# StefanHeng/Symbolic-Music-Generation

Measured on AMD Instinct MI355X. Metric: train tokens/sec (TransfoXL seq2048 bf16), whole job, higher is better.
Workload: dtype bf16; 1 GPU; TransfoXL 12L/768d H12 dh64 F3072 T=2048 M=2048 V=1190 cutoffs=[] (SURVEY C3, mode R: fresh zero mems); per_gpu_batch=64, global_batch=64, seq_len=2048, mem_len=2048, parallelism=dp1

## Files before the change

symbolic_music_generation_amd/csrc/relattn_fwd.hip:

```cpp
#include <type_traits>
#include "common.h"
#include "musicxl_internal.h"

namespace {

typedef __attribute__((ext_vector_type(8))) __bf16 mfma_bf16x8;
typedef __attribute__((address_space(3))) bf16x4 lds_bf16x4;

struct RelAttnP {
    const bf16_t *q, *k, *v, *rd;
    const float *rwb, *rrb;
    bf16_t* out;
    float* lse;
    int B, T, H, M, Kc;
    long long q_bs, kv_bs, o_bs;
    int q_rs, kv_rs, rd_rs, o_rs;
    float scale_log2e;
    bf16_t* oph;
    float* mph;
    int oph_all;
    char* ph_rec;
};

constexpr int QB = 128;
constexpr int KT = 64;
constexpr int GS = 100;
constexpr float NEG_BIG = -1.0e30f;

__device__ __forceinline__ int floordiv(int a, int b) { return (a >= 0) ? a / b : -((-a + b - 1) / b); }

template <int DH> struct Geo {
    static constexpr int KS = DH / 16;
    static constexpr int EB = (DH + 31) / 32;
    static constexpr int VW = EB * 32;
    static constexpr int ROWB = DH * 2;
    static constexpr int VROWB = VW * 2;
    static constexpr int CH = DH / 8;
    static constexpr int VCH = VW / 8;
    static constexpr int K_BYTES = KT * ROWB;
    static constexpr int V_BYTES = KT * VROWB;
    static constexpr int R_BYTES = 256 * ROWB;
    static constexpr int G_BYTES = 4 * 32 * GS * 2;
    static constexpr int SMEM = K_BYTES + V_BYTES + R_BYTES + G_BYTES;
    static constexpr int NLD_K = (KT * CH + 255) / 256;
    static constexpr int NLD_V = (KT * CH + 255) / 256;
    __device__ static __forceinline__ int koff(int row, int ch) {
        if (DH == 64) return row * ROWB + ((ch ^ ((row >> 1) & 7)) << 4);
        return row * ROWB + (ch << 4);
    }
    __device__ static __forceinline__ int eoff(int row, int e) { return koff(row, e >> 3) + ((e & 7) << 1); }
    __device__ static __forceinline__ int voff(int row, int byte) {
        if (DH == 64) return row * VROWB + (byte ^ (((row >> 1) & 1) << 6));
        return row * VROWB + byte;
    }
};

typedef _Float16 f16x4 __attribute__((ext_vector_type(4)));
typedef float f32x4v __attribute__((ext_vector_type(4)));


#define MXL_SKEW_READS                                                                                                        \
        "ds_read_u16 %0, %16 offset:54\n\t"  "ds_read_u16 %1, %16 offset:52\n\t"  "ds_read_u16 %2, %16 offset:50\n\t"           \
        "ds_read_u16 %3, %16 offset:48\n\t"  "ds_read_u16 %4, %16 offset:38\n\t"  "ds_read_u16 %5, %16 offset:36\n\t"           \
        "ds_read_u16 %6, %16 offset:34\n\t"  "ds_read_u16 %7, %16 offset:32\n\t"  "ds_read_u16 %8, %16 offset:22\n\t"           \
        "ds_read_u16 %9, %16 offset:20\n\t"  "ds_read_u16 %10, %16 offset:18\n\t" "ds_read_u16 %11, %16 offset:16\n\t"          \
        "ds_read_u16 %12, %16 offset:6\n\t"  "ds_read_u16 %13, %16 offset:4\n\t"  "ds_read_u16 %14, %16 offset:2\n\t"           \
        "ds_read_u16 %15, %16\n\t"
#define MXL_SKEW_OPERANDS                                                                                                     \
        : "=&v"(u[0]), "=&v"(u[1]), "=&v"(u[2]), "=&v"(u[3]), "=&v"(u[4]), "=&v"(u[5]), "=&v"(u[6]), "=&v"(u[7]),               \
          "=&v"(u[8]), "=&v"(u[9]), "=&v"(u[10]), "=&v"(u[11]), "=&v"(u[12]), "=&v"(u[13]), "=&v"(u[14]), "=&v"(u[15])          \
        : "v"(base)                                                                                                           \
        : "memory"
__device__ __forceinline__ void skew_issue16(uint32_t base, uint32_t (&u)[16]) {
    asm volatile(MXL_SKEW_READS "s_nop 0" MXL_SKEW_OPERANDS);
}
__device__ __forceinline__ void skew_issue16_w15(uint32_t base, uint32_t (&u)[16]) {
    asm volatile(MXL_SKEW_READS "s_waitcnt lgkmcnt(15)" MXL_SKEW_OPERANDS);
}
__device__ __forceinline__ void lgkm_wait0() { asm volatile("s_waitcnt lgkmcnt(0)" ::: "memory"); }

__device__ __forceinline__ float add_f16v(float s, uint32_t h16) {
    float r;
    asm volatile("v_fma_mix_f32 %0, %1, 1.0, %2 op_sel_hi:[0,0,1]" : "=v"(r) : "v"(s), "v"(h16));
    return r;
}

__device__ __forceinline__ float max3(float a, float b, float c) {
    float r;
    asm("v_max3_f32 %0, %1, %2, %3" : "=v"(r) : "v"(a), "v"(b), "v"(c));
    return r;
}

#ifdef MXL_STAMP
__device__ unsigned long long g_fwd_stamps[16];
#define STAMP_DECL unsigned long long st_last, st_acc[16] = {0ull, 0ull, 0ull, 0ull, 0ull, 0ull, 0ull, 0ull, 0ull, 0ull, 0ull, 0ull, 0ull, 0ull, 0ull, 0ull}; \
    { __builtin_amdgcn_sched_barrier(0); asm volatile("s_memtime %0\n\ts_waitcnt lgkmcnt(0)" : "=s"(st_last) :: "memory"); __builtin_amdgcn_sched_barrier(0); }
#define STAMP(i) { unsigned long long t_; __builtin_amdgcn_sched_barrier(0); asm volatile("s_memtime %0\n\ts_waitcnt lgkmcnt(0)" : "=s"(t_) :: "memory"); \
    __builtin_amdgcn_sched_barrier(0); st_acc[i] += t_ - st_last; st_last = t_; }
#define STAMP_FLUSH if ((threadIdx.x & 63) == 0) { for (int i_ = 0; i_ < 16; i_++) atomicAdd(&g_fwd_stamps[i_], st_acc[i_]); }
#else
#define STAMP_DECL
#define STAMP(i)
#define STAMP_FLUSH
#endif

#ifndef FWD_PRIO
#define FWD_PRIO 6
#endif
#define FPRIO_UP(bit_) do { if (FWD_PRIO & (bit_)) __builtin_amdgcn_s_setprio(1); } while (0)
#define FPRIO_DOWN(bit_) do { if (FWD_PRIO & (bit_)) __builtin_amdgcn_s_setprio(0); } while (0)
constexpr float RESCALE_THRESH = 8.0f;
constexpr float FAST_SUM_MAX = 8192.0f;

template <int DH>
__global__ __launch_bounds__(256, 2) void relattn_fwd_kernel(RelAttnP p) {
    using G = Geo<DH>;
    constexpr int KS = G::KS, EB = G::EB;
    extern __shared__ __attribute__((aligned(16))) char smem[];
    char* sK = smem;
    char* sV = sK + G::K_BYTES;
    char* sR = sV + G::V_BYTES;
    _Float16* sG = reinterpret_cast<_Float16*>(sR + G::R_BYTES);

    STAMP_DECL
    const int tid = threadIdx.x;
    const int wid = __builtin_amdgcn_readfirstlane(tid >> 6);
    const int l = tid & 63, r = l & 31, hh = l >> 5;
    int bx_, h, b;
    xcd_block(bx_, h, b);
    const int i0 = (gridDim.x - 1 - bx_) * QB;
    const int iw0 = i0 + 32 * wid;
    const int T = p.T, M = p.M;
    const int p0 = T - p.Kc;
    _Float16* gW = sG + wid * 32 * GS + r * GS + 4 * hh;
    const _Float16* gR = sG + wid * 32 * GS + r * GS + r + 64 - 4 * hh;
    const uint32_t gRb = (uint32_t)(uintptr_t)(__attribute__((address_space(3))) const char*)(const char*)(gR - 27);
    f16x4 carry[4];
    int rfr[KS];
#pragma unroll
    for (int ks = 0; ks < KS; ks++)
        rfr[ks] = r * G::ROWB + ((DH == 64) ? (((2 * ks + hh) ^ ((r >> 1) & 7)) << 4) : ((2 * ks + hh) << 4));

    const bf16_t* kbase = p.k + (size_t)b * p.kv_bs + (size_t)h * DH;
    const bf16_t* vbase = p.v + (size_t)b * p.kv_bs + (size_t)h * DH;
    const bf16_t* rbase = p.rd + (size_t)h * DH;

    bf16x8 qw[KS], qr[KS];
    {
        const int i = iw0 + r;
        const bool ok = i < T;
        const bf16_t* qp = p.q + (size_t)b * p.q_bs + (size_t)(ok ? i : 0) * p.q_rs + (size_t)h * DH;
#pragma unroll
        for (int ks = 0; ks < KS; ks++) {
            const int e0 = 16 * ks + 8 * hh;
            bf16x8 qv = *reinterpret_cast<const bf16x8*>(qp + e0);
#pragma unroll
            for (int j = 0; j < 8; j++) {
                const float qf = ok ? bf2f((bf16_t)qv[j]) : 0.f;
                qw[ks][j] = (short)f2bf((qf + p.rwb[h * DH + e0 + j]) * p.scale_log2e);
                qr[ks][j] = (short)f2bf((qf + p.rrb[h * DH + e0 + j]) * p.scale_log2e);
            }
        }
    }

    if (p.ph_rec && iw0 < T) {
        char* rec = p.ph_rec + (((size_t)b * p.H + h) * (size_t)(T >> 5) + (iw0 >> 5)) * 4352;
        const int sw = (((r >> 1) & 1) << 2) | (((r >> 2) & 1) << 1) | ((r >> 3) & 1);
#pragma unroll
        for (int ks = 0; ks < KS; ks++) *reinterpret_cast<bf16x8*>(rec + r * 128 + (((2 * ks + hh) ^ sw) << 4)) = qr[ks];
    }

    const int p_lo = i0 - M + 1;
    const int p_hi = min(i0 + QB - 1, T - 1);
    const int kt_lo = floordiv(p_lo, KT), kt_hi = floordiv(p_hi, KT);

    typedef u32x4 stage_t[G::NLD_K];
    stage_t rk, rv, rr[2];
    const unsigned kv_bytes = (unsigned)(((long long)(p.Kc - 1) * p.kv_rs + DH) * 2);
    const unsigned rd_bytes = (unsigned)(((long long)(M - 1) * p.rd_rs + DH) * 2);
    const __amdgpu_buffer_rsrc_t rs_k = __builtin_amdgcn_make_buffer_rsrc((void*)kbase, 0, (int)kv_bytes, 0x00020000);
    const __amdgpu_buffer_rsrc_t rs_v = __builtin_amdgcn_make_buffer_rsrc((void*)vbase, 0, (int)kv_bytes, 0x00020000);
    const __amdgpu_buffer_rsrc_t rs_r = __builtin_amdgcn_make_buffer_rsrc((void*)rbase, 0, (int)rd_bytes, 0x00020000);
    constexpr bool STG_ALL = (KT * G::CH) % 256 == 0;
    int kvo[G::NLD_K], rdo[G::NLD_K], kst[G::NLD_K], vst[G::NLD_K];
#pragma unroll
    for (int n = 0; n < G::NLD_K; n++) {
        const int c = tid + n * 256;
        const int row = c / G::CH, ch = c % G::CH;
        kvo[n] = ((row - p0) * p.kv_rs + ch * 8) * 2;
        rdo[n] = (row * p.rd_rs + ch * 8) * 2;
        kst[n] = G::koff(row & (KT - 1), ch);
        vst[n] = G::voff(row & (KT - 1), ch * 16);
    }
    auto load_kv = [&](stage_t& dk, stage_t& dv, int P) __attribute__((always_inline)) {
        const int so = P * p.kv_rs * 2;
#pragma unroll
        for (int n = 0; n < G::NLD_K; n++) {
            if (STG_ALL || tid + n * 256 < KT * G::CH) {
                dk[n] = __builtin_bit_cast(u32x4, __builtin_amdgcn_raw_buffer_load_b128(rs_k, kvo[n] + so, 0, 0));
                dv[n] = __builtin_bit_cast(u32x4, __builtin_amdgcn_raw_buffer_load_b128(rs_v, kvo[n] + so, 0, 0));
            } else {
                dk[n] = u32x4{0u, 0u, 0u, 0u}; dv[n] = u32x4{0u, 0u, 0u, 0u};
            }
        }
    };
    auto store_kv = [&](const stage_t& sk, const stage_t& sv) __attribute__((always_inline)) {
#pragma unroll
        for (int n = 0; n < G::NLD_K; n++) {
            if (STG_ALL || tid + n * 256 < KT * G::CH) {
                *reinterpret_cast<u32x4*>(sK + kst[n]) = sk[n];
                *reinterpret_cast<u32x4*>(sV + vst[n]) = sv[n];
            }
        }
    };
    auto load_r = [&](stage_t& dst, int dbase) __attribute__((always_inline)) {
        const int so = dbase * p.rd_rs * 2;
#pragma unroll
        for (int n = 0; n < G::NLD_K; n++) {
            if (STG_ALL || tid + n * 256 < KT * G::CH)
                dst[n] = __builtin_bit_cast(u32x4, __builtin_amdgcn_raw_buffer_load_b128(rs_r, rdo[n] + so, 0, 0));
            else dst[n] = u32x4{0u, 0u, 0u, 0u};
        }
    };
    auto store_r = [&](const stage_t& src, int dbase) __attribute__((always_inline)) {
        char* ring = sR + (dbase & 255) * G::ROWB;
#pragma unroll
        for (int n = 0; n < G::NLD_K; n++)
            if (STG_ALL || tid + n * 256 < KT * G::CH) *reinterpret_cast<u32x4*>(ring + kst[n]) = src[n];
    };

    if (DH < G::VW) {
        for (int i = tid; i < G::V_BYTES / 4; i += 256) reinterpret_cast<uint32_t*>(sV)[i] = 0u;
        __syncthreads();
    }

    float m_run = NEG_BIG, l_run = 0.f;
    bool all_set = false;
    f32x16 cinit;
#pragma unroll
    for (int j = 0; j < 16; j++) cinit[j] = 0.f;
    f32x16 o[EB];
#pragma unroll
    for (int e = 0; e < EB; e++)
#pragma unroll
        for (int j = 0; j < 16; j++) o[e][j] = 0.f;

    auto rebase = [&](f32x16 (&x)[2], auto&& rescale_acc, bool after_attempt, float rs_attempt) __attribute__((always_inline)) {
        float mx = NEG_BIG;
#pragma unroll
        for (int kb = 0; kb < 2; kb++)
#pragma unroll
            for (int j = 0; j < 16; j += 2) mx = max3(mx, x[kb][j], x[kb][j + 1]);
        mx = fmaxf(mx, __shfl_xor(mx, 32, 64));
        const bool unset = m_run == NEG_BIG;
        const float rs_other = __shfl_xor(rs_attempt, 32, 64);
        const bool bad_q = !(rs_attempt <= FAST_SUM_MAX) || !(rs_other <= FAST_SUM_MAX);
        const bool need = unset ? (mx > 0.5f * NEG_BIG) : (after_attempt ? bad_q : (mx > RESCALE_THRESH));
        if (__any(need)) {
            const float delta = need ? mx : 0.f;
            const float alpha = (need && !unset) ? __builtin_amdgcn_exp2f(-delta) : 1.f;
            if (need) m_run = (unset ? 0.f : m_run) + delta;
            const float neg = (m_run == NEG_BIG) ? 0.f : -m_run;
            l_run *= alpha;
#pragma unroll
            for (int j = 0; j < 16; j++) { x[0][j] -= delta; x[1][j] -= delta; cinit[j] = neg; }
            rescale_acc(alpha);
        }
        all_set = !__any(m_run == NEG_BIG);
    };
    auto exp_sum = [&](f32x16 (&x)[2]) __attribute__((always_inline)) {
        float rs = 0.f;
#pragma unroll
        for (int kb = 0; kb < 2; kb++)
#pragma unroll
            for (int j = 0; j < 16; j++) { x[kb][j] = __builtin_amdgcn_exp2f(x[kb][j]); rs += x[kb][j]; }
        return rs;
    };

    const int pz = floordiv(p0, KT) * KT;
    int kt_start = kt_lo;
    const int tk0 = G::eoff(4 * hh + ((l & 15) >> 2), 16 * ((l >> 4) & 1) + 4 * (l & 3));
    if (kt_lo * KT < pz) {
        kt_start = pz / KT;
        const int qi = iw0 + r;
        const int db0 = i0 - pz;
        load_r(rk, db0);
        load_r(rr[1], db0 + 64);
        load_r(rr[0], db0 + 128);
        store_r(rk, db0);
        __syncthreads();
        auto chunk = [&](auto par_, int db) __attribute__((always_inline)) {
            constexpr int NXT = 1 - decltype(par_)::value;
            STAMP(15)
            store_r(rr[NXT], db + 64);
            load_r(rr[NXT], db + 192);
            STAMP(10)
            bool on[2], fl[2];
#pragma unroll
            for (int gb = 0; gb < 2; gb++) {
                const int dblk = db + 32 * gb;
                on[gb] = (iw0 < T) && !(dblk + 31 <= iw0 - pz || dblk > M - 1);
                fl[gb] = on[gb] && (dblk >= iw0 + 31 - pz + 1) && (dblk + 31 <= M - 1) && (iw0 + 31 < T);
            }
            if (on[0] || on[1]) {
                f32x16 g[2];
                const char* rb = sR + (db & 255) * G::ROWB;
                auto ph_scores = [&]() __attribute__((always_inline)) {
                    bf16x8 ra[2][KS];
#pragma unroll
                    for (int gb = 0; gb < 2; gb++)
#pragma unroll
                        for (int ks = 0; ks < KS; ks++) ra[gb][ks] = *reinterpret_cast<const bf16x8*>(rb + gb * 32 * G::ROWB + rfr[ks]);
                    __builtin_amdgcn_sched_barrier(0);
                    g[0] = cinit; g[1] = cinit;
                    FPRIO_UP(4);
#pragma unroll
                    for (int ks = 0; ks < KS; ks++)
#pragma unroll
                        for (int gb = 0; gb < 2; gb++)
                            g[gb] = __builtin_amdgcn_mfma_f32_32x32x16_bf16(__builtin_bit_cast(mfma_bf16x8, ra[gb][ks]),
                                                                            __builtin_bit_cast(mfma_bf16x8, qr[ks]), g[gb], 0, 0, 0);
                    FPRIO_DOWN(4);
#pragma unroll
                    for (int gb = 0; gb < 2; gb++) {
                        if (!fl[gb]) {
                            const int dblk = db + 32 * gb;
#pragma unroll
                            for (int j = 0; j < 16; j++) {
                                const int d = dblk + (j & 3) + 8 * (j >> 2) + 4 * hh;
                                const bool valid = (d >= qi - pz + 1) && (d <= M - 1) && (qi < T);
                                g[gb][j] = valid ? g[gb][j] : NEG_BIG;
                            }
                        }
                    }
                };
                auto rescale_oph = [&](float alpha) __attribute__((always_inline)) {
                    if (p.oph) {
#pragma unroll
                        for (int e = 0; e < EB; e++)
#pragma unroll
                            for (int j = 0; j < 16; j++) o[e][j] *= alpha;
                    }
                };
                const bool attempt = all_set;
                bool precise = !attempt, bad = false;
                float rs = 0.f;
                if (attempt) {
                    ph_scores();
                    STAMP(11)
                    rs = exp_sum(g);
                    bad = !(rs <= FAST_SUM_MAX);
                    precise = __any(bad);
                }
                if (precise) {
                    ph_scores();
                    rebase(g, rescale_oph, attempt, rs);
                    rs = exp_sum(g);
                }
                l_run += rs;
                STAMP(12)
                FPRIO_UP(4);
#pragma unroll
                for (int gb = 0; gb < 2; gb++) {
                    const int dblk = db + 32 * gb;
                    if (p.oph && on[gb] && (p.oph_all || (dblk & ~255) > iw0 + 31 - pz)) {
                        const int gq = l >> 4, li = l & 15, q4 = li >> 2, pp = li & 3;
                        const char* rbb = rb + gb * 32 * G::ROWB;
#pragma unroll
                        for (int st = 0; st < 2; st++) {
                            const u32x4 pw = {pack2bf(g[gb][8 * st], g[gb][8 * st + 1]), pack2bf(g[gb][8 * st + 2], g[gb][8 * st + 3]),
                                              pack2bf(g[gb][8 * st + 4], g[gb][8 * st + 5]), pack2bf(g[gb][8 * st + 6], g[gb][8 * st + 7])};
                            const bf16x8 pf = __builtin_bit_cast(bf16x8, pw);
#pragma unroll
                            for (int e = 0; e < EB; e++) {
                                const int dist = dblk + 16 * st + 4 * hh + q4;
                                const int ecol = 32 * e + 16 * (gq & 1) + 4 * pp;
                                bf16x8 a = {0, 0, 0, 0, 0, 0, 0, 0};
                                if (DH == 64) {
                                    const char* a0 = rbb + tk0 + 16 * st * G::ROWB;
                                    const bf16x4 lo = __builtin_amdgcn_ds_read_tr16_b64_v4i16((lds_bf16x4*)(a0 + 64 * e));
                                    const bf16x4 hi = __builtin_amdgcn_ds_read_tr16_b64_v4i16((lds_bf16x4*)(a0 + 8 * G::ROWB + 64 * (1 - e)));
                                    a = bf16x8{lo[0], lo[1], lo[2], lo[3], hi[0], hi[1], hi[2], hi[3]};
                                } else if (ecol < DH) {
                                    const bf16x4 lo = __builtin_amdgcn_ds_read_tr16_b64_v4i16((lds_bf16x4*)(sR + G::eoff(dist & 255, ecol)));
                                    const bf16x4 hi = __builtin_amdgcn_ds_read_tr16_b64_v4i16((lds_bf16x4*)(sR + G::eoff((dist + 8) & 255, ecol)));
                                    a = bf16x8{lo[0], lo[1], lo[2], lo[3], hi[0], hi[1], hi[2], hi[3]};
                                }
                                o[e] = __builtin_amdgcn_mfma_f32_32x32x16_bf16(__builtin_bit_cast(mfma_bf16x8, a),
                                                                               __builtin_bit_cast(mfma_bf16x8, pf), o[e], 0, 0, 0);
                            }
                        }
                    }
                }
                FPRIO_DOWN(4);
            }
            STAMP(13)
            __syncthreads();
            STAMP(14)
        };
#pragma unroll 1
        for (int db = db0; db <= M - 1; db += 128) {
            chunk(std::integral_constant<int, 0>{}, db);
            if (db + 64 > M - 1) break;
            chunk(std::integral_constant<int, 1>{}, db + 64);
        }
    }

    if (p.oph) {
        const int qi = iw0 + r;
        if (qi < T) {
            bf16_t* op = p.oph + (size_t)b * p.o_bs + (size_t)qi * p.o_rs + (size_t)h * DH;
#pragma unroll
            for (int e = 0; e < EB; e++) {
#pragma unroll
                for (int grp = 0; grp < 4; grp++) {
                    const int e0 = 32 * e + 8 * grp + 4 * hh;
                    if (e0 < DH) {
                        u32x2 w = {pack2bf(o[e][4 * grp], o[e][4 * grp + 1]), pack2bf(o[e][4 * grp + 2], o[e][4 * grp + 3])};
                        *reinterpret_cast<u32x2*>(op + e0) = w;
                    }
                }
            }
            if (hh == 0) p.mph[((size_t)b * p.H + h) * T + qi] = (m_run == NEG_BIG) ? 0.f : m_run;
        }
#pragma unroll
        for (int e = 0; e < EB; e++)
#pragma unroll
            for (int j = 0; j < 16; j++) o[e][j] = 0.f;
    }

    {
        const int P0 = kt_start * KT;
        const int dbase = i0 - P0 - 64;
        stage_t w2;
        load_kv(rk, rv, P0);
        load_r(rr[0], dbase);
        load_r(rr[1], dbase + 64);
        load_r(w2, dbase + 128);
        store_kv(rk, rv);
        store_r(rr[0], dbase);
        store_r(rr[1], dbase + 64);
        store_r(w2, dbase + 128);
    }
    __syncthreads();

    bool have_ring = false;
    auto rescale_o = [&](float alpha) __attribute__((always_inline)) {
#pragma unroll
        for (int e = 0; e < EB; e++)
#pragma unroll
            for (int j = 0; j < 16; j++) o[e][j] *= alpha;
    };

#pragma unroll 1
    for (int kt = kt_start; kt <= kt_hi; kt++) {
        const int P = kt * KT;
        STAMP(15)
        load_kv(rk, rv, P + KT);
        load_r(rr[0], i0 - (P + KT) - 64);
        STAMP(0)
        const int dmin_w = iw0 - P - (KT - 1), dmax_w = iw0 + 31 - P;
        const bool active = (dmax_w >= 0) && (dmin_w <= M - 1) && (iw0 < T);
        if (active) {
            const char* cK = sK;
            const char* cV = sV;
            const int dlo = iw0 - P - 64;
            auto gblock = [&](int gb, f16x4 (&dst)[4]) __attribute__((always_inline)) {
                f32x16 g;
#pragma unroll
                for (int j = 0; j < 16; j++) g[j] = 0.f;
                const char* rb = sR + ((dlo + 32 * gb) & 255) * G::ROWB;
#pragma unroll
                for (int ks = 0; ks < KS; ks++) {
                    const bf16x8 a = *reinterpret_cast<const bf16x8*>(rb + rfr[ks]);
                    g = __builtin_amdgcn_mfma_f32_32x32x16_bf16(__builtin_bit_cast(mfma_bf16x8, a),
                                                                __builtin_bit_cast(mfma_bf16x8, qr[ks]), g, 0, 0, 0);
                }
#pragma unroll
                for (int grp = 0; grp < 4; grp++) {
                    const f32x4v v4 = {g[4 * grp], g[4 * grp + 1], g[4 * grp + 2], g[4 * grp + 3]};
                    dst[grp] = __builtin_convertvector(v4, f16x4);
                }
            };
            f16x4 b0[4], b1[4];
            if (!have_ring) gblock(2, carry);
            {
                bf16x8 ra[2][KS];
#pragma unroll
                for (int gb = 0; gb < 2; gb++) {
                    const char* rb = sR + ((dlo + 32 * gb) & 255) * G::ROWB;
#pragma unroll
                    for (int ks = 0; ks < KS; ks++) ra[gb][ks] = *reinterpret_cast<const bf16x8*>(rb + rfr[ks]);
                }
                __builtin_amdgcn_sched_barrier(0);
                f32x16 g0, g1;
#pragma unroll
                for (int j = 0; j < 16; j++) { g0[j] = 0.f; g1[j] = 0.f; }
                FPRIO_UP(1);
#pragma unroll
                for (int ks = 0; ks < KS; ks++) {
                    g0 = __builtin_amdgcn_mfma_f32_32x32x16_bf16(__builtin_bit_cast(mfma_bf16x8, ra[0][ks]),
                                                                 __builtin_bit_cast(mfma_bf16x8, qr[ks]), g0, 0, 0, 0);
                    g1 = __builtin_amdgcn_mfma_f32_32x32x16_bf16(__builtin_bit_cast(mfma_bf16x8, ra[1][ks]),
                                                                 __builtin_bit_cast(mfma_bf16x8, qr[ks]), g1, 0, 0, 0);
                }
                FPRIO_DOWN(1);
                STAMP(1)
#pragma unroll
                for (int grp = 0; grp < 4; grp++) {
                    const f32x4v v0 = {g0[4 * grp], g0[4 * grp + 1], g0[4 * grp + 2], g0[4 * grp + 3]};
                    const f32x4v v1 = {g1[4 * grp], g1[4 * grp + 1], g1[4 * grp + 2], g1[4 * grp + 3]};
                    b0[grp] = __builtin_convertvector(v0, f16x4);
                    b1[grp] = __builtin_convertvector(v1, f16x4);
                }
            }
#pragma unroll
            for (int grp = 0; grp < 4; grp++) {
                *reinterpret_cast<f16x4*>(gW + 8 * grp) = b0[grp];
                *reinterpret_cast<f16x4*>(gW + 32 + 8 * grp) = b1[grp];
                *reinterpret_cast<f16x4*>(gW + 64 + 8 * grp) = carry[grp];
                carry[grp] = b0[grp];
            }
            have_ring = true;
            STAMP(2)
            const bool full = (dmin_w >= 0) && (dmax_w <= M - 1) && (iw0 + 31 < T);
            const int qi = iw0 + r;
            f32x16 s[2];
            auto tile_scores = [&](auto masked) __attribute__((always_inline)) {
                constexpr bool MASKED = decltype(masked)::value;
                {
                    bf16x8 ka[2][KS];
#pragma unroll
                    for (int kb = 0; kb < 2; kb++)
#pragma unroll
                        for (int ks = 0; ks < KS; ks++)
                            ka[kb][ks] = *reinterpret_cast<const bf16x8*>(cK + G::koff(32 * kb + r, 2 * ks + hh));
                    __builtin_amdgcn_sched_barrier(0);
                    s[0] = cinit; s[1] = cinit;
                    FPRIO_UP(1);
#pragma unroll
                    for (int ks = 0; ks < KS; ks++) {
#pragma unroll
                        for (int kb = 0; kb < 2; kb++)
                            s[kb] = __builtin_amdgcn_mfma_f32_32x32x16_bf16(__builtin_bit_cast(mfma_bf16x8, ka[kb][ks]),
                                                                            __builtin_bit_cast(mfma_bf16x8, qw[ks]), s[kb], 0, 0, 0);
                    }
                    FPRIO_DOWN(1);
                    __builtin_amdgcn_sched_barrier(0);
                }
                STAMP(3)
                uint32_t u0[16], u1[16];
                skew_issue16(gRb, u0);
                skew_issue16_w15(gRb - 64, u1);
#pragma unroll
                for (int kb = 0; kb < 2; kb++) {
                    if (kb == 1) lgkm_wait0();
#pragma unroll
                    for (int j = 0; j < 16; j++) {
                        float val = add_f16v(s[kb][j], kb == 0 ? u0[j] : u1[j]);
                        if (MASKED) {
                            const int d = qi - P - (32 * kb + (j & 3) + 8 * (j >> 2) + 4 * hh);
                            const bool valid = (d >= 0) && (d <= M - 1) && (qi < T);
                            val = valid ? val : NEG_BIG;
                        }
                        s[kb][j] = val;
                    }
                }
            };
            auto scores = [&]() __attribute__((always_inline)) { if (full) tile_scores(std::false_type{}); else tile_scores(std::true_type{}); };
            const bool attempt = all_set;
            bool precise = !attempt, bad = false;
            float rs = 0.f;
            if (attempt) {
                scores();
                STAMP(4)
                rs = exp_sum(s);
                bad = !(rs <= FAST_SUM_MAX);
                precise = __any(bad);
            }
            if (precise) {
                scores();
                rebase(s, rescale_o, attempt, rs);
                rs = exp_sum(s);
            }
            l_run += rs;
            STAMP(5)
            FPRIO_UP(2);
#pragma unroll
            for (int kb = 0; kb < 2; kb++) {
#pragma unroll
                for (int st = 0; st < 2; st++) {
                    const u32x4 pw = {pack2bf(s[kb][8 * st], s[kb][8 * st + 1]), pack2bf(s[kb][8 * st + 2], s[kb][8 * st + 3]),
                                      pack2bf(s[kb][8 * st + 4], s[kb][8 * st + 5]), pack2bf(s[kb][8 * st + 6], s[kb][8 * st + 7])};
                    const bf16x8 pf = __builtin_bit_cast(bf16x8, pw);
                    const int gq = l >> 4, li = l & 15, q4 = li >> 2, pp = li & 3;
#pragma unroll
                    for (int e = 0; e < EB; e++) {
                        const int key = 32 * kb + 16 * st + 4 * hh + q4;
                        const int byte = (32 * e + 16 * (gq & 1) + 4 * pp) * 2;
                        const lds_bf16x4* a0 = (const lds_bf16x4*)(cV + G::voff(key, byte));
                        const lds_bf16x4* a1 = (const lds_bf16x4*)(cV + G::voff(key + 8, byte));
                        const bf16x4 lo = __builtin_amdgcn_ds_read_tr16_b64_v4i16((lds_bf16x4*)a0);
                        const bf16x4 hi = __builtin_amdgcn_ds_read_tr16_b64_v4i16((lds_bf16x4*)a1);
                        const bf16x8 a = {lo[0], lo[1], lo[2], lo[3], hi[0], hi[1], hi[2], hi[3]};
                        o[e] = __builtin_amdgcn_mfma_f32_32x32x16_bf16(__builtin_bit_cast(mfma_bf16x8, a),
                                                                       __builtin_bit_cast(mfma_bf16x8, pf), o[e], 0, 0, 0);
                    }
                }
            }
            FPRIO_DOWN(2);
        }
        STAMP(6)
        __syncthreads();
        STAMP(7)
        store_kv(rk, rv);
        store_r(rr[0], i0 - (P + KT) - 64);
        STAMP(8)
        __syncthreads();
        STAMP(9)
    }
    STAMP(15)

    const float l_tot = l_run + __shfl_xor(l_run, 32, 64);
    const float inv = l_tot > 0.f ? 1.f / l_tot : 0.f;
    const int qi = iw0 + r;
    if (qi < T) {
        bf16_t* op = p.out + (size_t)b * p.o_bs + (size_t)qi * p.o_rs + (size_t)h * DH;
#pragma unroll
        for (int e = 0; e < EB; e++) {
#pragma unroll
            for (int grp = 0; grp < 4; grp++) {
                const int e0 = 32 * e + 8 * grp + 4 * hh;
                if (e0 < DH) {
                    u32x2 w = {pack2bf(o[e][4 * grp] * inv, o[e][4 * grp + 1] * inv),
                               pack2bf(o[e][4 * grp + 2] * inv, o[e][4 * grp + 3] * inv)};
                    *reinterpret_cast<u32x2*>(op + e0) = w;
                }
            }
        }
        const float lse2 = m_run + __builtin_amdgcn_logf(l_tot);
        if (hh == 0 && p.lse) p.lse[((size_t)b * p.H + h) * T + qi] = lse2 * 0.6931471805599453f;
        if (hh == 0 && p.ph_rec)
            reinterpret_cast<float*>(p.ph_rec + (((size_t)b * p.H + h) * (size_t)(T >> 5) + (iw0 >> 5)) * 4352 + 4096)[r] = -lse2;
    }
    STAMP(15)
    STAMP_FLUSH
}

template <int DH>
int launch_fwd(const RelAttnP& p, hipStream_t s) {
    using G = Geo<DH>;
    static bool attr_set = false;
    if (!attr_set) {
        hipError_t e = hipFuncSetAttribute(reinterpret_cast<const void*>(&relattn_fwd_kernel<DH>),
                                           hipFuncAttributeMaxDynamicSharedMemorySize, G::SMEM);
        if (e != hipSuccess) return (int)e;
        attr_set = true;
    }
    dim3 grid((p.T + QB - 1) / QB, p.H, p.B);
    {
        mxl_kt::Scope kt(MXL_KT_RELATTN_FWD, s);
        hipLaunchKernelGGL((relattn_fwd_kernel<DH>), grid, dim3(256), G::SMEM, s, p);
    }
    MXL_LAUNCH_CHECK();
    return MXL_OK;
}

}

#ifdef MXL_STAMP
extern "C" int mxl_debug_fwd_stamps(unsigned long long* host_out16) {
    hipError_t e = hipMemcpyFromSymbol(host_out16, HIP_SYMBOL(g_fwd_stamps), sizeof(unsigned long long) * 16);
    if (e != hipSuccess) return (int)e;
    unsigned long long z[16] = {0};
    e = hipMemcpyToSymbol(HIP_SYMBOL(g_fwd_stamps), z, sizeof(z));
    return (int)e;
}
#endif

static int relattn_fwd_launch(const void* q, const void* k, const void* v, const void* rd, const float* r_w_bias,
                              const float* r_r_bias, void* out, float* lse, int B, int T, int H, int dh, int M, int Kc,
                              long long q_bs, int q_rs, long long kv_bs, int kv_rs, int rd_rs, long long o_bs, int o_rs,
                              float scale, void* oph, float* mph, void* stream, int oph_all = 0, void* ph_ws = nullptr) {
    MXL_CHECK_ARG(q && k && v && rd && r_w_bias && r_r_bias && out);
    if (oph_all) MXL_CHECK_ARG(oph && ((T - Kc) % 64) == 0);
    if (ph_ws) MXL_CHECK_ARG(oph_all && dh == 64 && ((uintptr_t)ph_ws % 16) == 0);
    if (oph) MXL_CHECK_ARG(mph && (M % (oph_all ? 32 : 256)) == 0 && (T % 32) == 0 && ((uintptr_t)oph % 8) == 0);
    MXL_CHECK_ARG(B > 0 && T > 0 && H > 0 && M > 0 && Kc >= T && Kc <= M + T);
    MXL_CHECK_ARG((q_rs % 8) == 0 && (kv_rs % 8) == 0 && (rd_rs % 8) == 0 && (o_rs % 4) == 0);
    MXL_CHECK_ARG((q_bs % 8) == 0 && (kv_bs % 8) == 0 && (o_bs % 4) == 0);
    MXL_CHECK_ARG((long long)Kc * kv_rs * 2 < (1ll << 31) && (long long)M * rd_rs * 2 < (1ll << 31));
    MXL_CHECK_ARG(((uintptr_t)q % 16) == 0 && ((uintptr_t)k % 16) == 0 && ((uintptr_t)v % 16) == 0 &&
                  ((uintptr_t)rd % 16) == 0 && ((uintptr_t)out % 8) == 0);
    RelAttnP p;
    p.q = (const bf16_t*)q; p.k = (const bf16_t*)k; p.v = (const bf16_t*)v; p.rd = (const bf16_t*)rd;
    p.rwb = r_w_bias; p.rrb = r_r_bias; p.out = (bf16_t*)out; p.lse = lse;
    p.B = B; p.T = T; p.H = H; p.M = M; p.Kc = Kc;
    p.q_bs = q_bs; p.kv_bs = kv_bs; p.o_bs = o_bs; p.q_rs = q_rs; p.kv_rs = kv_rs; p.rd_rs = rd_rs; p.o_rs = o_rs;
    p.scale_log2e = scale * 1.4426950408889634f;
    p.oph = (bf16_t*)oph; p.mph = mph; p.oph_all = oph_all ? 1 : 0; p.ph_rec = (char*)ph_ws;
    hipStream_t s = (hipStream_t)stream;
    switch (dh) {
        case 16: return launch_fwd<16>(p, s);
        case 32: return launch_fwd<32>(p, s);
        case 64: return launch_fwd<64>(p, s);
        default: return MXL_EUNSUPPORTED;
    }
}

extern "C" int mxl_relattn_fwd(const void* q, const void* k, const void* v, const void* rd, const float* r_w_bias,
                               const float* r_r_bias, void* out, float* lse, int B, int T, int H, int dh, int M, int Kc,
                               long long q_bs, int q_rs, long long kv_bs, int kv_rs, int rd_rs, long long o_bs, int o_rs,
                               float scale, void* stream) {
    return relattn_fwd_launch(q, k, v, rd, r_w_bias, r_r_bias, out, lse, B, T, H, dh, M, Kc, q_bs, q_rs, kv_bs, kv_rs, rd_rs, o_bs,
                              o_rs, scale, nullptr, nullptr, stream);
}

extern "C" int mxl_relattn_fwd_phantom(const void* q, const void* k, const void* v, const void* rd, const float* r_w_bias,
                                       const float* r_r_bias, void* out, float* lse, void* oph, float* mph, int B, int T, int H,
                                       int dh, int M, int Kc, long long q_bs, int q_rs, long long kv_bs, int kv_rs, int rd_rs,
                                       long long o_bs, int o_rs, float scale, void* stream) {
    MXL_CHECK_ARG(oph && mph);
    return relattn_fwd_launch(q, k, v, rd, r_w_bias, r_r_bias, out, lse, B, T, H, dh, M, Kc, q_bs, q_rs, kv_bs, kv_rs, rd_rs, o_bs,
                              o_rs, scale, oph, mph, stream);
}

extern "C" int mxl_relattn_fwd_phantom2(const void* q, const void* k, const void* v, const void* rd, const float* r_w_bias,
                                        const float* r_r_bias, void* out, float* lse, void* oph, float* mph, int oph_all, void* ph_ws,
                                        int B, int T, int H, int dh, int M, int Kc, long long q_bs, int q_rs, long long kv_bs, int kv_rs,
                                        int rd_rs, long long o_bs, int o_rs, float scale, void* stream) {
    MXL_CHECK_ARG(oph && mph);
    return relattn_fwd_launch(q, k, v, rd, r_w_bias, r_r_bias, out, lse, B, T, H, dh, M, Kc, q_bs, q_rs, kv_bs, kv_rs, rd_rs, o_bs,
                              o_rs, scale, oph, mph, stream, oph_all, ph_ws);
}
```

Before: 815,400 tokens/s.

## Add DMA-fed 8-wave relattn forward kernel with triple-buffered K/V

Adds a V2 variant of the relative-attention forward kernel for dh=64. It uses 512 threads (8 waves, 256 query rows per block) and loads K, V and R directly from global memory into LDS with buffer_load_lds instead of going through registers. K/V are triple-buffered and the R ring grows to 384 rows, so each tile needs one barrier plus a vmcnt wait instead of two syncthreads. Batched ds_read_b64_tr_b16 transposed reads feed the PV and phantom MFMAs. This removes register staging and a barrier per tile, at the cost of more LDS per block, which can lower occupancy, and fewer blocks in the grid. V2 is the default when T is a multiple of 256, and MXL_FWD_V1=1 selects the old kernel.

```diff
diff --git a/symbolic_music_generation_amd/csrc/relattn_fwd.hip b/symbolic_music_generation_amd/csrc/relattn_fwd.hip
--- a/symbolic_music_generation_amd/csrc/relattn_fwd.hip
+++ b/symbolic_music_generation_amd/csrc/relattn_fwd.hip
@@ -22,7 +22,6 @@
     char* ph_rec;
 };
 
-constexpr int QB = 128;
 constexpr int KT = 64;
 constexpr int GS = 100;
 constexpr float NEG_BIG = -1.0e30f;
@@ -91,6 +90,29 @@
     return r;
 }
 
+typedef unsigned long long u64x2 __attribute__((ext_vector_type(2)));
+typedef __attribute__((address_space(3))) void* lptr_t;
+template <int O, bool XHI>
+__device__ __forceinline__ void tr_read4x2(uint32_t x, uint32_t y, bf16x8 (&fa)[2][2]) {
+    u64x2 v00, v01, v10, v11;
+    const uint32_t xh = XHI ? y : x, yh = XHI ? x : y;
+    asm volatile(
+        "ds_read_b64_tr_b16 %0, %8 offset:%12\n\tds_read_b64_tr_b16 %1, %10 offset:%13\n\t"
+        "ds_read_b64_tr_b16 %2, %9 offset:%12\n\tds_read_b64_tr_b16 %3, %11 offset:%13\n\t"
+        "ds_read_b64_tr_b16 %4, %8 offset:%14\n\tds_read_b64_tr_b16 %5, %10 offset:%15\n\t"
+        "ds_read_b64_tr_b16 %6, %9 offset:%14\n\tds_read_b64_tr_b16 %7, %11 offset:%15\n\t"
+        "s_waitcnt lgkmcnt(0)"
+        : "=&v"(v00.x), "=&v"(v00.y), "=&v"(v01.x), "=&v"(v01.y), "=&v"(v10.x), "=&v"(v10.y), "=&v"(v11.x), "=&v"(v11.y)
+        : "v"(x), "v"(y), "v"(xh), "v"(yh), "n"(O), "n"(O + 1024), "n"(O + 2048), "n"(O + 3072)
+        : "memory");
+    fa[0][0] = __builtin_bit_cast(bf16x8, v00); fa[0][1] = __builtin_bit_cast(bf16x8, v01);
+    fa[1][0] = __builtin_bit_cast(bf16x8, v10); fa[1][1] = __builtin_bit_cast(bf16x8, v11);
+}
+template <int N> __device__ __forceinline__ void dma_barrier() {
+    asm volatile("s_waitcnt vmcnt(%0) lgkmcnt(0)" :: "n"(N) : "memory");
+    __builtin_amdgcn_s_barrier();
+}
+
 #ifdef MXL_STAMP
 __device__ unsigned long long g_fwd_stamps[16];
 #define STAMP_DECL unsigned long long st_last, st_acc[16] = {0ull, 0ull, 0ull, 0ull, 0ull, 0ull, 0ull, 0ull, 0ull, 0ull, 0ull, 0ull, 0ull, 0ull, 0ull, 0ull}; \
@@ -112,15 +134,26 @@
 constexpr float RESCALE_THRESH = 8.0f;
 constexpr float FAST_SUM_MAX = 8192.0f;
 
-template <int DH>
-__global__ __launch_bounds__(256, 2) void relattn_fwd_kernel(RelAttnP p) {
+template <int DH, bool V2> struct FwdCfg {
+    static constexpr int NW = V2 ? 8 : 4;
+    static constexpr int QB = 32 * NW;
+    static constexpr int RR = V2 ? 384 : 256;
+    static constexpr int NKV = V2 ? 3 : 1;
+    static constexpr int SMEM = NKV * (Geo<DH>::K_BYTES + Geo<DH>::V_BYTES) + RR * Geo<DH>::ROWB + NW * 32 * GS * 2;
+};
+
+template <int DH, bool V2>
+__global__ __launch_bounds__(V2 ? 512 : 256, 2) void relattn_fwd_kernel(RelAttnP p) {
     using G = Geo<DH>;
-    constexpr int KS = G::KS, EB = G::EB;
-    extern __shared__ __attribute__((aligned(16))) char smem[];
+    using C = FwdCfg<DH, V2>;
+    static_assert(!V2 || DH == 64, "the DMA-fed form is written for 128-byte rows");
+    constexpr int KS = G::KS, EB = G::EB, QB = C::QB;
+    extern __shared__ __attribute__((aligned(1024))) char smem[];
     char* sK = smem;
-    char* sV = sK + G::K_BYTES;
-    char* sR = sV + G::V_BYTES;
-    _Float16* sG = reinterpret_cast<_Float16*>(sR + G::R_BYTES);
+    char* sV = sK + C::NKV * G::K_BYTES;
+    char* sR = sV + C::NKV * G::V_BYTES;
+    _Float16* sG = reinterpret_cast<_Float16*>(sR + C::RR * G::ROWB);
+    auto rslot = [](int d) __attribute__((always_inline)) { if (!V2) return d & 255; const int m = d % C::RR; return m < 0 ? m + C::RR : m; };
 
     STAMP_DECL
     const int tid = threadIdx.x;
@@ -223,11 +256,26 @@
         }
     };
     auto store_r = [&](const stage_t& src, int dbase) __attribute__((always_inline)) {
-        char* ring = sR + (dbase & 255) * G::ROWB;
+        char* ring = sR + rslot(dbase) * G::ROWB;
 #pragma unroll
         for (int n = 0; n < G::NLD_K; n++)
             if (STG_ALL || tid + n * 256 < KT * G::CH) *reinterpret_cast<u32x4*>(ring + kst[n]) = src[n];
     };
+
+    const int drow = 8 * wid + (l >> 3);
+    const int dchk = (l & 7) ^ ((drow >> 1) & 7), dchv = (l & 7) ^ (((drow >> 1) & 1) << 2);
+    const int dko = ((drow - p0) * p.kv_rs + dchk * 8) * 2, dvo = ((drow - p0) * p.kv_rs + dchv * 8) * 2;
+    const int dro = (drow * p.rd_rs + dchk * 8) * 2;
+    auto dma_kv = [&](int P, int buf) __attribute__((always_inline)) {
+        const int so = P * p.kv_rs * 2;
+        __builtin_amdgcn_raw_ptr_buffer_load_lds(rs_k, (lptr_t)(sK + buf * G::K_BYTES + wid * 1024), 16, dko + so, 0, 0, 0);
+        __builtin_amdgcn_raw_ptr_buffer_load_lds(rs_v, (lptr_t)(sV + buf * G::V_BYTES + wid * 1024), 16, dvo + so, 0, 0, 0);
+    };
+    auto dma_r = [&](int dbase) __attribute__((always_inline)) {
+        __builtin_amdgcn_raw_ptr_buffer_load_lds(rs_r, (lptr_t)(sR + rslot(dbase) * G::ROWB + wid * 1024), 16,
+                                                 dro + dbase * p.rd_rs * 2, 0, 0, 0);
+    };
+    const uint32_t lds0 = (uint32_t)(uintptr_t)(__attribute__((address_space(3))) char*)smem;
 
     if (DH < G::VW) {
         for (int i = tid; i < G::V_BYTES / 4; i += 256) reinterpret_cast<uint32_t*>(sV)[i] = 0u;
@@ -284,16 +332,25 @@
         kt_start = pz / KT;
         const int qi = iw0 + r;
         const int db0 = i0 - pz;
-        load_r(rk, db0);
-        load_r(rr[1], db0 + 64);
-        load_r(rr[0], db0 + 128);
-        store_r(rk, db0);
-        __syncthreads();
+        if (V2) {
+            dma_r(db0); dma_r(db0 + 64); dma_r(db0 + 128); dma_r(db0 + 192);
+            dma_barrier<3>();
+        } else {
+            load_r(rk, db0);
+            load_r(rr[1], db0 + 64);
+            load_r(rr[0], db0 + 128);
+            store_r(rk, db0);
+            __syncthreads();
+        }
         auto chunk = [&](auto par_, int db) __attribute__((always_inline)) {
             constexpr int NXT = 1 - decltype(par_)::value;
             STAMP(15)
-            store_r(rr[NXT], db + 64);
-            load_r(rr[NXT], db + 192);
+            if (V2) {
+                dma_r(db + 256);
+            } else {
+                store_r(rr[NXT], db + 64);
+                load_r(rr[NXT], db + 192);
+            }
             STAMP(10)
             bool on[2], fl[2];
 #pragma unroll
@@ -304,7 +361,7 @@
             }
             if (on[0] || on[1]) {
                 f32x16 g[2];
-                const char* rb = sR + (db & 255) * G::ROWB;
+                const char* rb = sR + rslot(db) * G::ROWB;
                 auto ph_scores = [&]() __attribute__((always_inline)) {
                     bf16x8 ra[2][KS];
 #pragma unroll
@@ -366,6 +423,11 @@
                     if (p.oph && on[gb] && (p.oph_all || (dblk & ~255) > iw0 + 31 - pz)) {
                         const int gq = l >> 4, li = l & 15, q4 = li >> 2, pp = li & 3;
                         const char* rbb = rb + gb * 32 * G::ROWB;
+                        bf16x8 fa[2][2];
+                        if (V2) {
+                            const uint32_t ab = lds0 + (uint32_t)(rbb - smem) + tk0;
+                            tr_read4x2<0, true>(ab, ab + 64, fa);
+                        }
 #pragma unroll
                         for (int st = 0; st < 2; st++) {
                             const u32x4 pw = {pack2bf(g[gb][8 * st], g[gb][8 * st + 1]), pack2bf(g[gb][8 * st + 2], g[gb][8 * st + 3]),
@@ -376,7 +438,9 @@
                                 const int dist = dblk + 16 * st + 4 * hh + q4;
                                 const int ecol = 32 * e + 16 * (gq & 1) + 4 * pp;
                                 bf16x8 a = {0, 0, 0, 0, 0, 0, 0, 0};
-                                if (DH == 64) {
+                                if (V2) {
+                                    a = fa[st][e];
+                                } else if (DH == 64) {
                                     const char* a0 = rbb + tk0 + 16 * st * G::ROWB;
                                     const bf16x4 lo = __builtin_amdgcn_ds_read_tr16_b64_v4i16((lds_bf16x4*)(a0 + 64 * e));
                                     const bf16x4 hi = __builtin_amdgcn_ds_read_tr16_b64_v4i16((lds_bf16x4*)(a0 + 8 * G::ROWB + 64 * (1 - e)));
@@ -395,7 +459,7 @@
                 FPRIO_DOWN(4);
             }
             STAMP(13)
-            __syncthreads();
+            if (V2) dma_barrier<3>(); else __syncthreads();
             STAMP(14)
         };
 #pragma unroll 1
@@ -429,7 +493,16 @@
             for (int j = 0; j < 16; j++) o[e][j] = 0.f;
     }
 
-    {
+    if (V2) {
+        const int P0 = kt_start * KT;
+        const int dbase = i0 - P0 - 64;
+        asm volatile("s_waitcnt vmcnt(0)" ::: "memory");
+        dma_kv(P0, 0);
+#pragma unroll
+        for (int j = 0; j < 5; j++) dma_r(dbase + 64 * j);
+        dma_kv(P0 + KT, 1);
+        dma_barrier<2>();
+    } else {
         const int P0 = kt_start * KT;
         const int dbase = i0 - P0 - 64;
         stage_t w2;
@@ -441,10 +514,11 @@
         store_r(rr[0], dbase);
         store_r(rr[1], dbase + 64);
         store_r(w2, dbase + 128);
-    }
-    __syncthreads();
+        __syncthreads();
+    }
 
     bool have_ring = false;
+    int cur = 0;
     auto rescale_o = [&](float alpha) __attribute__((always_inline)) {
 #pragma unroll
         for (int e = 0; e < EB; e++)
@@ -456,20 +530,25 @@
     for (int kt = kt_start; kt <= kt_hi; kt++) {
         const int P = kt * KT;
         STAMP(15)
-        load_kv(rk, rv, P + KT);
-        load_r(rr[0], i0 - (P + KT) - 64);
+        if (V2) {
+            dma_r(i0 - (P + KT) - 64);
+            dma_kv(P + 2 * KT, cur == 0 ? 2 : cur - 1);
+        } else {
+            load_kv(rk, rv, P + KT);
+            load_r(rr[0], i0 - (P + KT) - 64);
+        }
         STAMP(0)
         const int dmin_w = iw0 - P - (KT - 1), dmax_w = iw0 + 31 - P;
         const bool active = (dmax_w >= 0) && (dmin_w <= M - 1) && (iw0 < T);
         if (active) {
-            const char* cK = sK;
-            const char* cV = sV;
+            const char* cK = sK + (V2 ? cur * G::K_BYTES : 0);
+            const char* cV = sV + (V2 ? cur * G::V_BYTES : 0);
             const int dlo = iw0 - P - 64;
             auto gblock = [&](int gb, f16x4 (&dst)[4]) __attribute__((always_inline)) {
                 f32x16 g;
 #pragma unroll
                 for (int j = 0; j < 16; j++) g[j] = 0.f;
-                const char* rb = sR + ((dlo + 32 * gb) & 255) * G::ROWB;
+                const char* rb = sR + rslot(dlo + 32 * gb) * G::ROWB;
 #pragma unroll
                 for (int ks = 0; ks < KS; ks++) {
                     const bf16x8 a = *reinterpret_cast<const bf16x8*>(rb + rfr[ks]);
@@ -488,7 +567,7 @@
                 bf16x8 ra[2][KS];
 #pragma unroll
                 for (int gb = 0; gb < 2; gb++) {
-                    const char* rb = sR + ((dlo + 32 * gb) & 255) * G::ROWB;
+                    const char* rb = sR + rslot(dlo + 32 * gb) * G::ROWB;
 #pragma unroll
                     for (int ks = 0; ks < KS; ks++) ra[gb][ks] = *reinterpret_cast<const bf16x8*>(rb + rfr[ks]);
                 }
@@ -588,6 +667,12 @@
             FPRIO_UP(2);
 #pragma unroll
             for (int kb = 0; kb < 2; kb++) {
+                bf16x8 fa[2][2];
+                if (V2) {
+                    const int gq1 = (l >> 4) & 1, q4 = (l & 15) >> 2, pp = l & 3;
+                    const uint32_t vb = lds0 + (uint32_t)(cV - smem) + G::voff(4 * hh + q4, (16 * gq1 + 4 * pp) * 2);
+                    if (kb == 0) tr_read4x2<0, false>(vb, vb ^ 64u, fa); else tr_read4x2<4096, false>(vb, vb ^ 64u, fa);
+                }
 #pragma unroll
                 for (int st = 0; st < 2; st++) {
                     const u32x4 pw = {pack2bf(s[kb][8 * st], s[kb][8 * st + 1]), pack2bf(s[kb][8 * st + 2], s[kb][8 * st + 3]),
@@ -596,6 +681,11 @@
                     const int gq = l >> 4, li = l & 15, q4 = li >> 2, pp = li & 3;
 #pragma unroll
                     for (int e = 0; e < EB; e++) {
+                        if (V2) {
+                            o[e] = __builtin_amdgcn_mfma_f32_32x32x16_bf16(__builtin_bit_cast(mfma_bf16x8, fa[st][e]),
+                                                                           __builtin_bit_cast(mfma_bf16x8, pf), o[e], 0, 0, 0);
+                            continue;
+                        }
                         const int key = 32 * kb + 16 * st + 4 * hh + q4;
                         const int byte = (32 * e + 16 * (gq & 1) + 4 * pp) * 2;
                         const lds_bf16x4* a0 = (const lds_bf16x4*)(cV + G::voff(key, byte));
@@ -611,14 +701,21 @@
             FPRIO_DOWN(2);
         }
         STAMP(6)
-        __syncthreads();
-        STAMP(7)
-        store_kv(rk, rv);
-        store_r(rr[0], i0 - (P + KT) - 64);
-        STAMP(8)
-        __syncthreads();
-        STAMP(9)
-    }
+        if (V2) {
+            dma_barrier<2>();
+            cur = cur == 2 ? 0 : cur + 1;
+            STAMP(7)
+        } else {
+            __syncthreads();
+            STAMP(7)
+            store_kv(rk, rv);
+            store_r(rr[0], i0 - (P + KT) - 64);
+            STAMP(8)
+            __syncthreads();
+            STAMP(9)
+        }
+    }
+    if (V2) asm volatile("s_waitcnt vmcnt(0)" ::: "memory");
     STAMP(15)
 
     const float l_tot = l_run + __shfl_xor(l_run, 32, 64);
@@ -647,20 +744,20 @@
     STAMP_FLUSH
 }
 
-template <int DH>
+template <int DH, bool V2 = false>
 int launch_fwd(const RelAttnP& p, hipStream_t s) {
-    using G = Geo<DH>;
+    using C = FwdCfg<DH, V2>;
     static bool attr_set = false;
     if (!attr_set) {
-        hipError_t e = hipFuncSetAttribute(reinterpret_cast<const void*>(&relattn_fwd_kernel<DH>),
-                                           hipFuncAttributeMaxDynamicSharedMemorySize, G::SMEM);
+        hipError_t e = hipFuncSetAttribute(reinterpret_cast<const void*>(&relattn_fwd_kernel<DH, V2>),
+                                           hipFuncAttributeMaxDynamicSharedMemorySize, C::SMEM);
         if (e != hipSuccess) return (int)e;
         attr_set = true;
     }
-    dim3 grid((p.T + QB - 1) / QB, p.H, p.B);
+    dim3 grid((p.T + C::QB - 1) / C::QB, p.H, p.B);
     {
         mxl_kt::Scope kt(MXL_KT_RELATTN_FWD, s);
-        hipLaunchKernelGGL((relattn_fwd_kernel<DH>), grid, dim3(256), G::SMEM, s, p);
+        hipLaunchKernelGGL((relattn_fwd_kernel<DH, V2>), grid, dim3(64 * C::NW), C::SMEM, s, p);
     }
     MXL_LAUNCH_CHECK();
     return MXL_OK;
@@ -703,7 +800,11 @@
     switch (dh) {
         case 16: return launch_fwd<16>(p, s);
         case 32: return launch_fwd<32>(p, s);
-        case 64: return launch_fwd<64>(p, s);
+        case 64: {
+            const char* v1 = getenv("MXL_FWD_V1");
+            if ((T % FwdCfg<64, true>::QB) == 0 && !(v1 && v1[0] == '1')) return launch_fwd<64, true>(p, s);
+            return launch_fwd<64>(p, s);
+        }
         default: return MXL_EUNSUPPORTED;
     }
 }
```

Result: slower. 801,100 tokens/s (-1.8%).
